# jkflying/opencalibration

Measured on AMD Instinct MI355X. Metric: images/sec end-to-end (extract+match+relax) on synthetic aerial grid; LM iters/sec, higher is better.
Workload: dtype f32 (extract) + fp4 0/1 bits, f32 accumulate, exact (match) + f64 (RANSAC, relax)

## Files before the change

### include/ochip.h

```cpp
#ifndef OCHIP_H
#define OCHIP_H

#include <stddef.h>
#include <stdint.h>

#ifdef __cplusplus
extern "C"
{
#endif

#define OCHIP_OK 0
#define OCHIP_EINVAL (-1)
#define OCHIP_ENOMEM (-2)
#define OCHIP_EHIP (-3)
#define OCHIP_ENODEV (-4)
#define OCHIP_ESTATE (-5)

#define OCHIP_DESC_WORDS64 8
#define OCHIP_DESC_BITS 486
#define OCHIP_NO_SECOND 0xFFFFu

    typedef struct ochip_ctx ochip_ctx;

    typedef struct ochip_pair
// ... 53 lines not shown
    {
        uint8_t *records;
        float *response;
        uint32_t *slot;
        uint32_t *num_sparse;
        uint8_t *conflict;
        uint32_t *subset;
        uint32_t *num_subset;
        uint8_t *subset_conflict;
        double subset_spacing;
    } ochip_feature_lists;
    int ochip_akaze_features(ochip_ctx *ctx, const uint8_t *images_bgr, uint32_t n_images, int width, int height, uint32_t max_kp,
                             double nms_radius, uint32_t *counts, const ochip_feature_lists *lists, int *work_wh);
    int ochip_akaze_features_dev(ochip_ctx *ctx, const uint8_t *images_bgr_dev, uint32_t n_images, int width, int height,
                                 uint32_t max_kp, double nms_radius, uint32_t *counts, const ochip_feature_lists *lists, int *work_wh);
    int ochip_feature_lists_from_keypoints(ochip_ctx *ctx, const float *kp6, const uint64_t *desc, const uint32_t *counts, uint32_t n_images,
                            uint32_t max_kp, int work_w, int work_h, double scale, double nms_radius,
                            const ochip_feature_lists *out);

    int ochip_synth_views_alloc(ochip_ctx *ctx, uint32_t n_images, int width, int height, uint8_t **images_dev);
    void ochip_synth_views_free(ochip_ctx *ctx, uint8_t *images_dev);
    int ochip_synth_views_read(ochip_ctx *ctx, const uint8_t *images_dev, uint32_t index, int width, int height,
                               uint8_t *host_out);
    int ochip_synth_render_views(ochip_ctx *ctx, uint8_t *images_dev, uint32_t first_image, uint32_t n_images, int width,
                                 int height, const double *cams, const double *model3, const double *plane2,
                                 const double *lattice3, uint32_t seed);

    int ochip_upload_keypoints(ochip_ctx *ctx, uint32_t image_id, const double *xy, uint32_t n, const double *model8);

    int ochip_upload_batch(ochip_ctx *ctx, uint32_t n_images, const uint32_t *counts, const uint64_t *desc_all,
// ... 352 lines not shown
```

### opencalibration_amd/capi.py

```python
import ctypes as C
import os

import numpy as np

_HERE = os.path.dirname(os.path.abspath(__file__))
LIB_PATH = os.path.join(_HERE, "libochip.so")

K_MATCH, K_RANSAC, K_RELAX_EVAL, K_RELAX_SOLVE, K_AKAZE = 0, 1, 2, 3, 4
NO_SECOND = 0xFFFF

PAIR_DTYPE = np.dtype([("image_1", np.uint32), ("image_2", np.uint32)])
MATCH_DTYPE = np.dtype([("best_k", np.uint32), ("best_count", np.uint16), ("second_count", np.uint16)])
RANSAC_JOB_DTYPE = np.dtype([("image_1", np.uint32), ("image_2", np.uint32), ("n", np.uint32), ("rng_state", np.uint32),
                             ("match_offset", np.uint64), ("eval_offset", np.uint64)])
RANSAC_MATCH_DTYPE = np.dtype([("k1", np.uint32), ("k2", np.uint32), ("count", np.uint16), ("reserved", np.uint16)])
RANSAC_RESULT_DTYPE = np.dtype([("H", np.float64, (9,)), ("score", np.float64), ("iterations", np.uint32), ("n_inliers", np.uint32),
                                ("improvements", np.uint32), ("reserved", np.uint32)])

EXPORTS = [
    "ochip_ctx_create", "ochip_ctx_destroy", "ochip_ctx_sibling", "ochip_ctx_attachment", "ochip_akaze_progress", "ochip_ctx_set_priority", "ochip_last_error", "ochip_device_info", "ochip_synchronize",
    "ochip_descriptors_reserve", "ochip_upload_descriptors", "ochip_descriptor_count",
    "ochip_match_batch", "ochip_match_launch", "ochip_match_fetch",
    "ochip_upload_keypoints", "ochip_ransac_homography_batch", "ochip_refit_homography_batch", "ochip_ransac_epipolar_batch",
    "ochip_upload_batch", "ochip_host_alloc", "ochip_host_free", "ochip_akaze_batch", "ochip_akaze_batch_dev", "ochip_akaze_features", "ochip_akaze_features_dev", "ochip_feature_lists_from_keypoints",
    "ochip_synth_views_alloc", "ochip_synth_views_free", "ochip_synth_render_views", "ochip_synth_views_read",
    "ochip_relax_problem_create", "ochip_relax_problem_destroy", "ochip_relax_set_cameras_constant",
    "ochip_relax_solve", "ochip_relax_get_state", "ochip_relax_set_shard", "ochip_relax_evaluate",
    "ochip_plane_setup_create", "ochip_plane_setup_override", "ochip_plane_setup_blocks", "ochip_plane_setup_destroy",
    "ochip_plane_chain_create", "ochip_plane_chain_run", "ochip_plane_chain_destroy",
    "ochip_relaxg_problem_create", "ochip_relaxg_problem_destroy", "ochip_relaxg_set_structure_only", "ochip_relaxg_solve",
    "ochip_relaxg_get_state", "ochip_relaxg_evaluate", "ochip_relaxg_set_exchange",
    "ochip_relaxp_problem_create", "ochip_relaxp_problem_destroy", "ochip_relaxp_set_structure_only", "ochip_relaxp_solve",
    "ochip_relaxp_get_state",
    "ochip_profile_reset", "ochip_profile_get", "ochip_match_work", "ochip_relax_work", "ochip_relax_memory", "ochip_work_counters",
    "ochip_debug_fp64", "ochip_debug_std_sort", "ochip_debug_lm_step", "ochip_debug_homography_fit4", "ochip_match_sort", "ochip_ransac_homography_batch_sorted", "ochip_edge_lists",
    "ochip_dense_index_create", "ochip_dense_index_destroy", "ochip_dense_match", "ochip_dense_link", "ochip_dense_triangulate",
    "ochip_rccl_unique_id", "ochip_rccl_comm_create", "ochip_rccl_comm_destroy", "ochip_rccl_comm_stats",
    "ochip_rccl_relax_exchange",
    "ochip_ortho_mesh_create", "ochip_ortho_mesh_destroy", "ochip_ortho_dsm", "ochip_ortho_thumbnail", "ochip_ortho_layers",
# ... 517 lines not shown
```

### opencalibration_amd/csrc/akaze.hip

```cpp
#include "ctx.hpp"

#include <algorithm>
#include <cmath>
#include <limits>
#include <cstring>
#include <type_traits>
#include <vector>

namespace
{

struct level_info
{
    int octave, w, h, sigma_size;
    float esigma;
    size_t off;
    int tile_off, tiles_x;
    int mask_off;
    int sup_off, sup_tx;
};

__device__ __forceinline__ int clampi(int v, int lo, int hi)
{
    return v < lo ? lo : (v > hi ? hi : v);
// ... 2621 lines not shown
            const float bx = x0 + ((float)(ci + di) + 0.5f + 0.6f * (hashf(id) - 0.5f)) * spacing;
            const float by = y0 + ((float)(cj + dj) + 0.5f + 0.6f * (hashf(id + 1) - 0.5f)) * spacing;
            const float amp = (0.25f + 0.5f * hashf(id + 2)) * ((hash32(id + 3) & 1) ? 1.0f : -1.0f);
            const float sg = spacing * (0.10f + 0.14f * hashf(id + 4));
            const float r2 = (gx - bx) * (gx - bx) + (gy - by) * (gy - by);
            v += amp * __expf(-r2 / (2.0f * sg * sg));
        }
    const float o = fminf(255.0f, fmaxf(0.0f, v * 255.0f));
    const uint8_t g = (uint8_t)o;
    uint8_t *p = out + ((size_t)blockIdx.z * w * h + (size_t)y * w + x) * 3;
    p[0] = g;
    p[1] = g;
    p[2] = g;
}

int akaze_run(ochip_ctx *ctx, const uint8_t *images_bgr, bool on_device, uint32_t n_images, int width, int height,
              uint32_t max_kp, float *kp6, uint64_t *desc, uint32_t *counts, int *work_wh,
              const ochip_feature_lists *lists = nullptr, double nms_radius = 8.0);

}

extern "C"
{

int ochip_akaze_batch(ochip_ctx *ctx, const uint8_t *images_bgr, uint32_t n_images, int width, int height,
                      uint32_t max_kp, float *kp6, uint64_t *desc, uint32_t *counts, int *work_wh)
{
    return akaze_run(ctx, images_bgr, false, n_images, width, height, max_kp, kp6, desc, counts, work_wh);
}

int ochip_akaze_batch_dev(ochip_ctx *ctx, const uint8_t *images_bgr_dev, uint32_t n_images, int width, int height,
                          uint32_t max_kp, float *kp6, uint64_t *desc, uint32_t *counts, int *work_wh)
{
    return akaze_run(ctx, images_bgr_dev, true, n_images, width, height, max_kp, kp6, desc, counts, work_wh);
}

int ochip_akaze_features(ochip_ctx *ctx, const uint8_t *images_bgr, uint32_t n_images, int width, int height, uint32_t max_kp,
                         double nms_radius, uint32_t *counts, const ochip_feature_lists *lists, int *work_wh)
// ... 173 lines not shown
        for (int k = 0; k < 16; k += 4)
            chains.push_back({2, 13 + k, -10 + (k / 4) * 5, -10, 0});
        for (size_t cidx = 0; cidx < chains.size(); cidx++)
            for (int ch = 0; ch < 3; ch++)
            {
                const ch_t &cc = chains[cidx];
                const unsigned int p0 = (unsigned int)((cc.i + 10) * 21 + (cc.j + 10));
                T.chain[3 * cidx + ch] = p0 | ((unsigned int)ch << 9) | ((unsigned int)cc.cls << 11) |
                                         ((unsigned int)cc.first_cell << 13) | ((unsigned int)cc.follows << 18);
            }
        return T;
    }();
    return G;
}

int akaze_run(ochip_ctx *ctx, const uint8_t *images_bgr, bool on_device, uint32_t n_images, int width, int height,
              uint32_t max_kp, float *kp6, uint64_t *desc, uint32_t *counts, int *work_wh, const ochip_feature_lists *lists,
              double nms_radius)
{
    if (!ctx || !counts || (n_images && (!images_bgr || (!lists && (!kp6 || !desc)))))
        return OCHIP_EINVAL;
    if (width <= 0 || height <= 0)
        return ochip_fail(ctx, OCHIP_EINVAL, "bad image size %d x %d", width, height);
    OCHIP_HIP(ctx, hipSetDevice(ctx->device));
    hipStream_t st = ctx->stream;
    const double scale = std::min(1.f, float(1600) / (float)std::max(width, height));
    const int W = (int)std::lrint(width * scale), H = (int)std::lrint(height * scale);
    if (work_wh)
    {
        work_wh[0] = W;
        work_wh[1] = H;
    }
    for (uint32_t i = 0; i < n_images; i++)
        counts[i] = 0;
    if (n_images == 0)
        return OCHIP_OK;
// ... 67 lines not shown
    unsigned char *d_dead = nullptr, *d_valid = nullptr;
    unsigned long long *d_desc = nullptr, *d_descc = nullptr;
    float *d_kpc = nullptr;
    unsigned int *d_counts = nullptr, *d_tile_counts = nullptr, *d_tile_base = nullptr, *d_tile_seq = nullptr;
    unsigned long long *d_mask = nullptr, *d_vmask = nullptr, *d_kmask = nullptr, *d_pmask = nullptr, *d_rmask = nullptr;
    unsigned int *d_found = nullptr;
    unsigned int *d_level_first = nullptr;
    unsigned int *d_turns = nullptr, *d_waiting = nullptr;
    unsigned int *d_wbase = nullptr, *d_live = nullptr, *d_nlive = nullptr;
    gather_tab *d_gtab = nullptr;
    const size_t src_px = (size_t)width * height;
    auto tiles = [&](int w, int h) { return dim3(8 * ((((w + BT_X - 1) / BT_X) * ((h + BT_Y - 1) / BT_Y) + 7) / 8), 1, B); };
    auto det_tiles = [&](int w, int h) { return dim3(8 * ((((w + BT_X - 1) / BT_X) * ((h + DT_Y - 1) / DT_Y) + 7) / 8), 1, B); };
    const dim3 tiles0 = tiles(W, H);
    const int n_tiles0 = ((W + BT_X - 1) / BT_X) * ((H + BT_Y - 1) / BT_Y);
    if (on_device)
        d_bgr = const_cast<uint8_t *>(images_bgr);
    else
        AK(up(ctx, allocs, &d_bgr, images_bgr, (size_t)B * src_px * 3));
    AK(up<uint8_t>(ctx, allocs, &d_gray, nullptr, (size_t)B * src_px + 4));
    AK(up<float>(ctx, allocs, &d_img, nullptr, (size_t)B * plane0));
    AK(up<float>(ctx, allocs, &d_flow, nullptr, (size_t)B * plane0));
    AK(up<float>(ctx, allocs, &d_ping, nullptr, (size_t)B * plane0));
    AK(up<unsigned int>(ctx, allocs, &d_pmax, nullptr, (size_t)B * n_tiles0));
    AK(up<float>(ctx, allocs, &d_Lt, nullptr, (size_t)B * img_stride));
    AK(up<float2>(ctx, allocs, &d_Lxy, nullptr, (size_t)B * img_stride));
    AK(up<float2>(ctx, allocs, &d_Fit, nullptr, (size_t)B * img_stride));
    AK(up<float>(ctx, allocs, &d_Rmax, nullptr, (size_t)B * img_stride));
    AK(up<float>(ctx, allocs, &d_kc, nullptr, B));
    AK(up<unsigned int>(ctx, allocs, &d_hmax, nullptr, B));
    AK(up<unsigned int>(ctx, allocs, &d_hist, nullptr, (size_t)B * 301));
    AK(up<unsigned int>(ctx, allocs, &d_ncand, nullptr, B));
    AK(up<cand_t>(ctx, allocs, &d_cands, nullptr, (size_t)B * max_cands));
    AK(up<unsigned char>(ctx, allocs, &d_dead, nullptr, (size_t)B * max_cands));
// ... 5 lines not shown
    AK(up<unsigned int>(ctx, allocs, &d_counts, nullptr, B));
    AK(up<unsigned int>(ctx, allocs, &d_tile_counts, nullptr, (size_t)B * n_tiles));
    AK(up<unsigned int>(ctx, allocs, &d_tile_base, nullptr, (size_t)B * n_tiles));
    AK(up<unsigned long long>(ctx, allocs, &d_mask, nullptr, (size_t)B * mask_stride));
    AK(up<unsigned long long>(ctx, allocs, &d_vmask, nullptr, (size_t)B * mask_stride));
    AK(up<unsigned long long>(ctx, allocs, &d_kmask, nullptr, (size_t)B * sup_stride));
    AK(up<unsigned long long>(ctx, allocs, &d_pmask, nullptr, (size_t)B * sup_stride));
    AK(up<unsigned long long>(ctx, allocs, &d_rmask, nullptr, (size_t)B * sup_stride));
    AK(up<unsigned int>(ctx, allocs, &d_turns, nullptr, (size_t)B * 2 * max_cands));
    AK(up<unsigned int>(ctx, allocs, &d_waiting, nullptr, (size_t)B * LV.n));
    AK(up<unsigned int>(ctx, allocs, &d_level_first, nullptr, (size_t)B * (LV.n + 1)));
    AK(up<unsigned int>(ctx, allocs, &d_found, nullptr, (size_t)B * max_cands));
    AK(up<unsigned int>(ctx, allocs, &d_wbase, nullptr, (size_t)B * mask_stride));
    AK(up<unsigned int>(ctx, allocs, &d_live, nullptr, (size_t)B * max_cands));
    AK(up<unsigned int>(ctx, allocs, &d_nlive, nullptr, B));
    {
        std::vector<std::pair<uint64_t, unsigned int>> keyed;
        keyed.reserve(n_tiles);
        auto spread = [](uint32_t v) {
            uint64_t x = v;
            x = (x | (x << 16)) & 0x0000FFFF0000FFFFull;
            x = (x | (x << 8)) & 0x00FF00FF00FF00FFull;
            x = (x | (x << 4)) & 0x0F0F0F0F0F0F0F0Full;
            x = (x | (x << 2)) & 0x3333333333333333ull;
            x = (x | (x << 1)) & 0x5555555555555555ull;
            return x;
        };
        for (int i = 0; i < LV.n; i++)
        {
            const level_info &l = LV.l[i];
            const int ty_n = (l.h + DT_Y - 1) / DT_Y;
            for (int ty = 0; ty < ty_n; ty++)
                for (int tx = 0; tx < l.tiles_x; tx++)
                    keyed.emplace_back(((uint64_t)i << 48) | spread((uint32_t)tx) | (spread((uint32_t)ty) << 1),
                                       (unsigned int)(l.tile_off + ty * l.tiles_x + tx));
        }
        std::sort(keyed.begin(), keyed.end());
        std::vector<unsigned int> seq(keyed.size());
        for (size_t i = 0; i < keyed.size(); i++)
            seq[i] = keyed[i].second;
        AK(up(ctx, allocs, &d_tile_seq, seq.data(), seq.size()));
    }
    {
        AK(up(ctx, allocs, &d_gtab, &host_gather_tab(), 1));
    }
    if (rc != OCHIP_OK)
    {
        cleanup();
        return rc;
    }
    auto grid2 = [&](int w, int h) { return dim3((w + 255) / 256, h, B); };
    auto taps_of = [](const std::vector<float> &k) {
        taps_t t{};
        t.n = (int)k.size();
        for (int i = 0; i < t.n && i < MAX_TAPS; i++)
            t.k[i] = k[i];
        return t;
    };
    const taps_t g1 = taps_of(gaussian_taps(1.0f)), g0 = taps_of(gaussian_taps(soffset));
    if (g1.n != 5 || g0.n != 9)
    {
        cleanup();
        return ochip_fail(ctx, OCHIP_EINVAL, "akaze: unexpected Gaussian kernel sizes %d / %d", g1.n, g0.n);
    }
    hipEvent_t e0, e1;
    ochip_prof_begin(ctx, OCHIP_K_AKAZE, &e0, &e1);

    const size_t n_px = (size_t)B * src_px;
    const bool resized = !(W == width && H == height);
    area_tab tx, ty;
    bool staged = false;
    if (resized)
    {
        tx = area_table(width, W, 1.0 / scale);
        ty = area_table(height, H, 1.0 / scale);
        staged = width % 4 == 0;
        for (int x0 = 0; x0 < W && staged; x0 += 256)
        {
            const int x1 = std::min(x0 + 256, W);
            const int c0 = tx.si[tx.off[x0]] & ~3, c1 = tx.si[tx.off[x1] - 1];
            staged = c1 - c0 + 1 <= RS_PITCH - 3;
            for (int x = x0; x < x1 && staged; x++)
                staged = tx.off[x + 1] - tx.off[x] <= RESIZE_MAX_TAPS;
        }
        for (int y0 = 0; y0 < H && staged; y0 += RESIZE_ROWS)
        {
            const int y1 = std::min(y0 + RESIZE_ROWS, H);
            staged = ty.si[ty.off[y1] - 1] - ty.si[ty.off[y0]] + 1 <= RS_ROWS;
        }
    }
    const bool fused_grey = staged && ((uintptr_t)d_bgr & 3) == 0;
    if (!fused_grey)
    {
        if (((uintptr_t)d_bgr & 3) == 0)
            hipLaunchKernelGGL(gray4_kernel, dim3((unsigned)(((n_px + 3) / 4 + 255) / 256)), dim3(256), 0, st,
                               (const uint32_t *)d_bgr, (uint32_t *)d_gray, n_px / 4);
        if (((uintptr_t)d_bgr & 3) != 0 || (n_px & 3))
        {
            const size_t first = ((uintptr_t)d_bgr & 3) ? 0 : (n_px & ~(size_t)3);
            hipLaunchKernelGGL(gray_kernel, dim3((unsigned)((n_px - first + 255) / 256)), dim3(256), 0, st, d_bgr + 3 * first,
                               d_gray + first, n_px - first);
        }
    }
    if (W == width && H == height)
        hipLaunchKernelGGL(to_float_kernel, dim3((unsigned)((B * plane0 + 255) / 256)), dim3(256), 0, st, d_gray, d_img,
                           B * plane0);
    else
    {
        int *xo, *xs, *yo, *ys;
        float *xa, *ya;
        AK(up(ctx, allocs, &xo, tx.off.data(), tx.off.size()));
        AK(up(ctx, allocs, &xs, tx.si.data(), tx.si.size()));
        AK(up(ctx, allocs, &xa, tx.alpha.data(), tx.alpha.size()));
        AK(up(ctx, allocs, &yo, ty.off.data(), ty.off.size()));
        AK(up(ctx, allocs, &ys, ty.si.data(), ty.si.size()));
        AK(up(ctx, allocs, &ya, ty.alpha.data(), ty.alpha.size()));
        if (rc != OCHIP_OK)
        {
            cleanup();
            return rc;
        }
        const dim3 rgrid((W + 255) / 256, (H + RESIZE_ROWS - 1) / RESIZE_ROWS, B);
        int most_taps = 0;
        for (int x = 0; x < W; x++)
            most_taps = std::max(most_taps, tx.off[x + 1] - tx.off[x]);
        const int half_up_cols = scale == 0.5 ? W - W % 16 : 0;
        if (fused_grey && most_taps <= 4)
            hipLaunchKernelGGL((resize_area_lds_kernel<true, 4>), rgrid, dim3(256), 0, st, (const uint8_t *)d_bgr, width, height, d_img,
                               W, H, xo, xs, xa, yo, ys, ya, half_up_cols);
        else if (fused_grey)
            hipLaunchKernelGGL((resize_area_lds_kernel<true, RESIZE_MAX_TAPS>), rgrid, dim3(256), 0, st, (const uint8_t *)d_bgr, width, height, d_img,
                               W, H, xo, xs, xa, yo, ys, ya, half_up_cols);
        else if (staged)
            hipLaunchKernelGGL((resize_area_lds_kernel<false, RESIZE_MAX_TAPS>), rgrid, dim3(256), 0, st, d_gray, width, height, d_img, W, H, xo, xs,
                               xa, yo, ys, ya, half_up_cols);
        else
            hipLaunchKernelGGL(resize_area_kernel, rgrid, dim3(256), 0, st, d_gray, width, height, d_img, W, H, xo, xs, xa, yo, ys,
                               ya, half_up_cols);
    }

// ... 302 lines not shown
            {
                std::fwrite(which ? hx.data() : hl.data(), 4, which ? hx.size() : hl.size(), f);
                std::fclose(f);
            }
    }
    hipLaunchKernelGGL(scan_tiles_kernel, dim3(B), dim3(256), 0, st, (const unsigned int *)d_tile_counts,
                       (const unsigned int *)d_tile_seq, n_tiles, d_tile_base, d_ncand);
    hipLaunchKernelGGL(collect_tiles_kernel, dim3((n_tiles + 4 * COLLECT_TPW - 1) / (4 * COLLECT_TPW), 1, B), dim3(256), 0, st, (const float *)d_Rmax,
                       (const float2 *)d_Fit, img_stride,
                       (const unsigned long long *)d_mask, mask_stride, LV, (const unsigned int *)d_tile_base, n_tiles, d_cands,
                       max_cands, (const unsigned int *)d_tile_counts);
    std::vector<unsigned int> ncand(B);
    OCHIP_HIP(ctx, hipMemcpyAsync(ncand.data(), d_ncand, B * 4, hipMemcpyDeviceToHost, st));
    OCHIP_HIP(ctx, ochip_stream_wait(ctx, st));
    ctx->akaze_readbacks.fetch_add(1, std::memory_order_release);
    unsigned int max_n = 0;
    for (uint32_t b = 0; b < B; b++)
    {
        if (ncand[b] > max_cands)
        {
            cleanup();
            return ochip_fail(ctx, OCHIP_ENOMEM, "image %u has %u extrema candidates; raise max_kp (candidate capacity %u)", b,
                              ncand[b], max_cands);
        }
        max_n = std::max(max_n, ncand[b]);
    }
    const int xcd_remap = 2;
    if (max_n > 0)
    {
        OCHIP_HIP(ctx, hipMemsetAsync(d_vmask, 0, (size_t)B * mask_stride * 8, st));
// ... 95 lines not shown
        if (counts[b] > max_kp)
        {
            rc = ochip_fail(ctx, OCHIP_ENOMEM, "image %u has %u keypoints, more than max_kp = %u", b, counts[b], max_kp);
            break;
        }
        most = std::max(most, counts[b]);
    }
    if (rc == OCHIP_OK && lists)
        rc = ochip::feature_lists_enqueue(ctx, &allocs, B, max_kp, d_kpc, d_descc, d_counts, most, W, H, scale, nms_radius, lists);
    else if (rc == OCHIP_OK && most > 0)
    {
        OCHIP_HIP(ctx, hipMemcpy2DAsync(kp6, (size_t)max_kp * 24, d_kpc, (size_t)max_kp * 24, (size_t)most * 24, B, hipMemcpyDeviceToHost, st));
        OCHIP_HIP(ctx, hipMemcpy2DAsync(desc, (size_t)max_kp * 64, d_descc, (size_t)max_kp * 64, (size_t)most * 64, B, hipMemcpyDeviceToHost, st));
    }
    if (rc != OCHIP_OK)
        for (uint32_t b = 0; b < B; b++)
            counts[b] = 0;
    cleanup();
    return rc;
#undef AK
}

}
```

### opencalibration_amd/csrc/ctx.hip

```cpp
#include "ctx.hpp"

#include <cstring>

static std::string g_create_error;

int ochip_fail(ochip_ctx *ctx, int code, const char *fmt, ...)
{
    char buf[512];
    va_list ap;
    va_start(ap, fmt);
    vsnprintf(buf, sizeof buf, fmt, ap);
    va_end(ap);
    if (ctx)
        ctx->error = buf;
    else
        g_create_error = buf;
    return code;
}

int ochip_ensure(ochip_ctx *ctx, void **ptr, size_t *cap, size_t bytes)
{
    if (bytes <= *cap)
        return OCHIP_OK;
    if (*ptr)
// ... 183 lines not shown
    for (void *b : bufs)
        if (b)
            (void)hipFree(b);
    for (void *b : ctx->scratch_dev)
        if (b)
            (void)hipFree(b);
    if (ctx->sym_jobs_dev)
        (void)hipFree(ctx->sym_jobs_dev);
    if (ctx->sym_part_dev)
        (void)hipFree(ctx->sym_part_dev);
    for (void *b : {ctx->desc_fp4_dev, ctx->desc_negpop_dev, ctx->desc_pop_dev})
        if (b)
            (void)hipFree(b);
    for (auto &b : ctx->dev_pool)
        (void)hipFree(b.first);
    for (auto &b : ctx->pinned_pool)
        (void)hipHostFree(b.first);
    for (auto &b : ctx->pinned_live)
        (void)hipHostFree(b.first);
    if (ctx->sync_event)
        (void)hipEventDestroy(ctx->sync_event);
    for (hipStream_t r : ctx->retired_streams)
        (void)hipStreamDestroy(r);
    if (ctx->stream)
        (void)hipStreamDestroy(ctx->stream);
    if (ctx->copy_stream)
        (void)hipStreamDestroy(ctx->copy_stream);
    delete ctx;
}

int ochip_ctx_set_priority(ochip_ctx *ctx, int high)
{
    if (!ctx)
        return OCHIP_EINVAL;
    if (ctx->stream_priority == (high ? 1 : 0))
        return OCHIP_OK;
    OCHIP_HIP(ctx, hipSetDevice(ctx->device));
    int least = 0, greatest = 0;
    OCHIP_HIP(ctx, hipDeviceGetStreamPriorityRange(&least, &greatest));
    OCHIP_HIP(ctx, hipStreamSynchronize(ctx->stream));
    hipStream_t s = nullptr;
    OCHIP_HIP(ctx, hipStreamCreateWithPriority(&s, hipStreamNonBlocking, high ? greatest : least));
    ctx->retired_streams.push_back(ctx->stream);
    ctx->stream = s;
    ctx->stream_priority = high ? 1 : 0;
    return OCHIP_OK;
}

int ochip_ctx_sibling(ochip_ctx *ctx, uint32_t index, ochip_ctx **out)
{
    if (!ctx || !out)
// ... 329 lines not shown
```

### opencalibration_amd/csrc/ctx.hpp

```cpp
#pragma once

#include <hip/hip_runtime.h>

#include <atomic>
#include <cstdarg>
#include <cstdio>
#include <mutex>
#include <string>
#include <vector>

#include "../../include/ochip.h"
#include "env.hpp"

struct ochip_profile_slot
{
    std::vector<std::pair<hipEvent_t, hipEvent_t>> pending;
    std::vector<std::pair<hipEvent_t, hipEvent_t>> free_list;
    uint64_t launches = 0;
    double total_ms = 0;
};

struct ochip_ctx
{
    int device = 0;
// ... 34 lines not shown
    uint64_t match_out_total = 0;
    void *ms_recs_dev = nullptr, *ms_seg_dev = nullptr, *ms_flag_dev = nullptr;
    size_t ms_recs_cap = 0, ms_seg_cap = 0, ms_flag_cap = 0;
    uint32_t ms_pairs = 0;
    void *sym_jobs_dev = nullptr, *sym_part_dev = nullptr;
    size_t sym_jobs_cap = 0, sym_part_cap = 0;
    void *desc_fp4_dev = nullptr, *desc_negpop_dev = nullptr, *desc_pop_dev = nullptr;
    size_t desc_fp4_cap = 0, desc_negpop_cap = 0, desc_pop_cap = 0;
    uint64_t fp4_valid = 0;

    void *scratch_dev[8] = {nullptr};
    size_t scratch_cap[8] = {0};

    std::vector<std::pair<void *, size_t>> pinned_live, pinned_pool;
    std::vector<std::pair<void *, size_t>> dev_pool;

    ochip_profile_slot prof[OCHIP_K_COUNT];
    uint64_t match_computed = 0, match_delivered = 0;
    double relax_mfma_flops = 0;
    uint64_t ransac_hyp_corr = 0, relax_blocks_jac = 0, relax_blocks_cost = 0;
    uint64_t relax_system_bytes = 0, relax_system_dense_bytes = 0, relax_system_unknowns = 0;

    std::vector<ochip_ctx *> siblings;
    std::mutex siblings_mutex;

    std::atomic<uint64_t> akaze_readbacks{0};

    void *attachment = nullptr;
    void (*attachment_destroy)(void *) = nullptr;
};


inline hipError_t ochip_stream_wait(ochip_ctx *ctx, hipStream_t st)
{
    if (!ctx->blocking_wait)
        return hipStreamSynchronize(st);
    if (!ctx->sync_event)
    {
        const hipError_t e = hipEventCreateWithFlags(&ctx->sync_event, hipEventBlockingSync | hipEventDisableTiming);
        if (e != hipSuccess)
            return e;
// ... 45 lines not shown
```

### opencalibration_amd/csrc/env.hpp

```cpp
#pragma once

#include <cstdlib>
#include <cstring>

inline bool ochip_env_list_has(const char *var, const char *name, bool one_means_all)
{
    const char *e = std::getenv(var);
    if (!e || !*e)
        return false;
    if (one_means_all && (std::strcmp(e, "1") == 0 || std::strcmp(e, "all") == 0))
        return true;
    const size_t len = std::strlen(name);
    for (const char *p = e; *p;)
    {
        const char *q = std::strchr(p, ',');
        const size_t n = q ? (size_t)(q - p) : std::strlen(p);
        if (n == len && std::strncmp(p, name, len) == 0)
            return true;
        p += n + (q ? 1 : 0);
    }
    return false;
}
inline bool ochip_verbose(const char *what)
{
    return ochip_env_list_has("OCHIP_VERBOSE", what, true);
}
inline bool ochip_test_hook(const char *name)
{
    return ochip_env_list_has("OCHIP_TEST_HOOKS", name, false);
}
```

### opencalibration_amd/csrc/host/extract_features.cpp

```cpp
#include "../env.hpp"
#include "extract_features.hpp"
#include "extract_slots.hpp"
#include "sort_like_std.hpp"

#include <algorithm>
#include <chrono>
#include <cmath>
#include <condition_variable>
#include <cstdio>
#include <cstdlib>
#include <cstring>
#include <deque>
#include <limits>
#include <mutex>
#include <thread>

#include <emmintrin.h>
#include <omp.h>

namespace opencalibration_amd
{

namespace
{
// ... 447 lines not shown
            double &out, t0;
            ~at_exit() { out = thread_cpu_now() - t0; }
        } record{driver_cpu[d], cpu0};
        {
            slot_hold hold(slots, ticket.id(), d, handover);
            if (trace)
                fprintf(stderr, "[extract] survey %llu driver %u: slot acquired\n", (unsigned long long)ticket.id(), d);
            {
                std::lock_guard<std::mutex> lk(mu);
                if (!started)
                {
                    started = true;
                    t_first_slot = std::chrono::steady_clock::now();
                }
            }
            for (;;)
            {
                uint32_t c = 0;
                bool go = false;
                {
                    std::unique_lock<std::mutex> lk(mu);
                    if (stagger)
                        while (fail.empty() && next_chunk < n_chunks)
                        {
                            bool other = false;
                            for (uint32_t o = 0; o < n_drivers; o++)
                                if (o != d && in_first_phase[o])
                                {
                                    if (ochip_akaze_progress(ctxs[o]) != progress_at_start[o])
                                        in_first_phase[o] = 0;
// ... 9 lines not shown
                        c = next_chunk++;
                        go = true;
                        if (stagger)
                        {
                            progress_at_start[d] = ochip_akaze_progress(dctx);
                            in_first_phase[d] = 1;
                        }
                    }
                }
                if (!go)
                    break;
                if (c + 1 == n_chunks && handover == extract_slots::order::slot)
                    ticket.retire();
                if (trace)
                    fprintf(stderr, "[extract] survey %llu driver %u: chunk %u of %u\n", (unsigned long long)ticket.id(), d, c, n_chunks);
                const int sb = slots.take_buffer(d);
                const int which = BPS * (int)d + sb;
                chunk_buffers &b = bufs[which];
                int rc = OCHIP_OK;
                if (!shape_buffer(dctx, slots.at(d, sb), b))
                    rc = OCHIP_ENOMEM;
                b.first = c * chunk;
                b.n = std::min(chunk, n_images - b.first);
                int wh[2];
                const uint8_t *src = images_bgr + (size_t)b.first * image_bytes;
                if (rc != OCHIP_OK)
                    ;
                else if (device_tail)
                    rc = images_on_device ? ochip_akaze_features_dev(dctx, src, b.n, width, height, max_keypoints, nms_pixel_radius,
                                                                     b.counts.data(), &b.lists, wh)
                                          : ochip_akaze_features(dctx, src, b.n, width, height, max_keypoints, nms_pixel_radius,
                                                                 b.counts.data(), &b.lists, wh);
                else
                    rc = images_on_device ? ochip_akaze_batch_dev(dctx, src, b.n, width, height, max_keypoints, b.kp, b.desc,
                                                                  b.counts.data(), wh)
                                          : ochip_akaze_batch(dctx, src, b.n, width, height, max_keypoints, b.kp, b.desc,
                                                              b.counts.data(), wh);
                std::unique_lock<std::mutex> lk(mu);
                in_first_phase[d] = 0;
                if (rc != OCHIP_OK)
                {
                    if (fail.empty())
                        fail = std::string("ochip_akaze_batch: ") + ochip_last_error(dctx);
                    if (trace)
                        fprintf(stderr, "[extract] survey %llu driver %u: chunk %u failed (%s)\n", (unsigned long long)ticket.id(), d, c,
                                ochip_last_error(dctx));
                    lk.unlock();
                    cv.notify_all();
                    slots.return_buffer(d, sb);
                    ticket.retire();
                    break;
                }
                ready.push_back(which);
                cv.notify_all();
            }
        }
        if (trace)
            fprintf(stderr, "[extract] survey %llu driver %u: slot released\n", (unsigned long long)ticket.id(), d);
        std::unique_lock<std::mutex> lk(mu);
        drivers_done++;
        cv.notify_all();
    };
    std::vector<std::thread> drivers;
    for (uint32_t d = 0; d < n_drivers; d++)
        drivers.emplace_back(driver, d);
    std::chrono::steady_clock::time_point t_last_final = t_enter;

    for (;;)
    {
        int which;
// ... 123 lines not shown
```

### opencalibration_amd/csrc/host/extract_slots.hpp

```cpp
#pragma once

#include <condition_variable>
#include <cstddef>
#include <cstdint>
#include <mutex>
#include <set>

namespace opencalibration_amd
{

class extract_slots
{
  public:
    static constexpr uint32_t MAX_SLOTS = 8;
    static constexpr int BUFFERS_PER_SLOT = 3;
    enum class order
    {
        slot,
        survey,
        none
    };
    struct buffer
    {
        void *block[2] = {nullptr, nullptr};
// ... 49 lines not shown
    {
        std::unique_lock<std::mutex> lk(mu_);
        int b = -1;
        cv_.wait(lk, [&] {
            for (int i = 0; i < BUFFERS_PER_SLOT; i++)
                if (!slot_[d].buf[i].busy)
                {
                    b = i;
                    return true;
                }
            return false;
        });
        slot_[d].buf[b].busy = true;
        return b;
    }
    void return_buffer(uint32_t d, int b)
    {
        {
            std::lock_guard<std::mutex> lk(mu_);
            slot_[d].buf[b].busy = false;
        }
        cv_.notify_all();
    }
    buffer &at(uint32_t d, int b) { return slot_[d].buf[b]; }

  private:
    struct slot
    {
        bool held = false;
        uint64_t holder = 0;
// ... 44 lines not shown
```

Measured before the change: 3896.

## Split AKAZE extraction into begin/finish to overlap chunks and cache lookup tables

Extraction now runs in two steps. A begin call enqueues a chunk and records an event, and a finish call waits on that event later. This lets the host driver start the next chunk while the previous chunk's result copies are still draining. The tile-order sequence, gather table and resize tables are now cached on the context instead of being rebuilt and uploaded every batch, which removes per-chunk host sorting and small uploads. The cost is extra state: a pending-chunk limit, event recycling, and callback-driven collection, all of which raise the risk of ordering or buffer-lifetime bugs.

```diff
diff --git a/include/ochip.h b/include/ochip.h
--- a/include/ochip.h
+++ b/include/ochip.h
@@ -91,6 +91,12 @@
                              double nms_radius, uint32_t *counts, const ochip_feature_lists *lists, int *work_wh);
     int ochip_akaze_features_dev(ochip_ctx *ctx, const uint8_t *images_bgr_dev, uint32_t n_images, int width, int height,
                                  uint32_t max_kp, double nms_radius, uint32_t *counts, const ochip_feature_lists *lists, int *work_wh);
+    typedef struct ochip_akaze_job ochip_akaze_job;
+    int ochip_akaze_begin(ochip_ctx *ctx, const uint8_t *images_bgr, int images_on_device, uint32_t n_images, int width, int height,
+                          uint32_t max_kp, double nms_radius, float *kp6, uint64_t *desc, uint32_t *counts,
+                          const ochip_feature_lists *lists, int *work_wh, void (*stream_drained)(void *), void *arg,
+                          ochip_akaze_job **job);
+    int ochip_akaze_finish(ochip_ctx *ctx, ochip_akaze_job *job);
     int ochip_feature_lists_from_keypoints(ochip_ctx *ctx, const float *kp6, const uint64_t *desc, const uint32_t *counts, uint32_t n_images,
                             uint32_t max_kp, int work_w, int work_h, double scale, double nms_radius,
                             const ochip_feature_lists *out);
diff --git a/opencalibration_amd/capi.py b/opencalibration_amd/capi.py
--- a/opencalibration_amd/capi.py
+++ b/opencalibration_amd/capi.py
@@ -22,7 +22,7 @@
     "ochip_descriptors_reserve", "ochip_upload_descriptors", "ochip_descriptor_count",
     "ochip_match_batch", "ochip_match_launch", "ochip_match_fetch",
     "ochip_upload_keypoints", "ochip_ransac_homography_batch", "ochip_refit_homography_batch", "ochip_ransac_epipolar_batch",
-    "ochip_upload_batch", "ochip_host_alloc", "ochip_host_free", "ochip_akaze_batch", "ochip_akaze_batch_dev", "ochip_akaze_features", "ochip_akaze_features_dev", "ochip_feature_lists_from_keypoints",
+    "ochip_upload_batch", "ochip_host_alloc", "ochip_host_free", "ochip_akaze_batch", "ochip_akaze_batch_dev", "ochip_akaze_features", "ochip_akaze_features_dev", "ochip_akaze_begin", "ochip_akaze_finish", "ochip_feature_lists_from_keypoints",
     "ochip_synth_views_alloc", "ochip_synth_views_free", "ochip_synth_render_views", "ochip_synth_views_read",
     "ochip_relax_problem_create", "ochip_relax_problem_destroy", "ochip_relax_set_cameras_constant",
     "ochip_relax_solve", "ochip_relax_get_state", "ochip_relax_set_shard", "ochip_relax_evaluate",
diff --git a/opencalibration_amd/csrc/akaze.hip b/opencalibration_amd/csrc/akaze.hip
--- a/opencalibration_amd/csrc/akaze.hip
+++ b/opencalibration_amd/csrc/akaze.hip
@@ -2659,14 +2659,65 @@
     p[2] = g;
 }
 
+int akaze_begin(ochip_ctx *ctx, const uint8_t *images_bgr, bool on_device, uint32_t n_images, int width, int height,
+                uint32_t max_kp, float *kp6, uint64_t *desc, uint32_t *counts, int *work_wh, const ochip_feature_lists *lists,
+                double nms_radius, void (*stream_drained)(void *), void *arg, ochip_akaze_job **job);
+
 int akaze_run(ochip_ctx *ctx, const uint8_t *images_bgr, bool on_device, uint32_t n_images, int width, int height,
               uint32_t max_kp, float *kp6, uint64_t *desc, uint32_t *counts, int *work_wh,
-              const ochip_feature_lists *lists = nullptr, double nms_radius = 8.0);
-
-}
+              const ochip_feature_lists *lists = nullptr, double nms_radius = 8.0)
+{
+    ochip_akaze_job *job = nullptr;
+    const int rc = akaze_begin(ctx, images_bgr, on_device, n_images, width, height, max_kp, kp6, desc, counts, work_wh, lists,
+                               nms_radius, nullptr, nullptr, &job);
+    return rc != OCHIP_OK ? rc : ochip_akaze_finish(ctx, job);
+}
+
+}
+
+struct ochip_akaze_job
+{
+    hipEvent_t done = nullptr;
+    uint32_t *counts = nullptr;
+    uint32_t n_images = 0;
+};
 
 extern "C"
 {
+
+int ochip_akaze_begin(ochip_ctx *ctx, const uint8_t *images_bgr, int images_on_device, uint32_t n_images, int width, int height,
+                      uint32_t max_kp, double nms_radius, float *kp6, uint64_t *desc, uint32_t *counts,
+                      const ochip_feature_lists *lists, int *work_wh, void (*stream_drained)(void *), void *arg,
+                      ochip_akaze_job **job)
+{
+    if (!job)
+        return OCHIP_EINVAL;
+    *job = nullptr;
+    if (lists && (!lists->records || !lists->response || !lists->slot || !lists->num_sparse || !lists->conflict))
+        return OCHIP_EINVAL;
+    return akaze_begin(ctx, images_bgr, images_on_device != 0, n_images, width, height, max_kp, kp6, desc, counts, work_wh, lists,
+                       nms_radius, stream_drained, arg, job);
+}
+
+int ochip_akaze_finish(ochip_ctx *ctx, ochip_akaze_job *job)
+{
+    if (!ctx)
+        return OCHIP_EINVAL;
+    if (!job)
+        return OCHIP_OK;
+    const hipError_t e = hipEventSynchronize(job->done);
+    ctx->akaze_events.push_back(job->done);
+    ctx->akaze_pending--;
+    int rc = OCHIP_OK;
+    if (e != hipSuccess)
+    {
+        for (uint32_t b = 0; b < job->n_images; b++)
+            job->counts[b] = 0;
+        rc = ochip_fail(ctx, OCHIP_EHIP, "akaze: the chunk's result copies failed: %s", hipGetErrorString(e));
+    }
+    delete job;
+    return rc;
+}
 
 int ochip_akaze_batch(ochip_ctx *ctx, const uint8_t *images_bgr, uint32_t n_images, int width, int height,
                       uint32_t max_kp, float *kp6, uint64_t *desc, uint32_t *counts, int *work_wh)
@@ -2870,12 +2921,126 @@
     return G;
 }
 
-int akaze_run(ochip_ctx *ctx, const uint8_t *images_bgr, bool on_device, uint32_t n_images, int width, int height,
-              uint32_t max_kp, float *kp6, uint64_t *desc, uint32_t *counts, int *work_wh, const ochip_feature_lists *lists,
-              double nms_radius)
-{
+int akaze_tables_ensure(ochip_ctx *ctx, int width, int height, int W, int H, double scale, const levels_dev &LV, int n_tiles)
+{
+    auto &T = ctx->akaze_tab;
+    hipStream_t st = ctx->stream;
+    if (!T.gather)
+    {
+        void *g = nullptr;
+        if (hipMalloc(&g, sizeof(gather_tab)) != hipSuccess)
+            return ochip_fail(ctx, OCHIP_ENOMEM, "device allocation of %zu bytes failed in akaze", sizeof(gather_tab));
+        if (hipMemcpyAsync(g, &host_gather_tab(), sizeof(gather_tab), hipMemcpyHostToDevice, st) != hipSuccess ||
+            ochip_stream_wait(ctx, st) != hipSuccess)
+        {
+            (void)hipFree(g);
+            return ochip_fail(ctx, OCHIP_EHIP, "hipMemcpy failed in akaze");
+        }
+        T.gather = g;
+    }
+    if (T.block && T.width == width && T.height == height && T.W == W && T.H == H && T.n_tiles == n_tiles)
+        return OCHIP_OK;
+    OCHIP_HIP(ctx, ochip_stream_wait(ctx, st));
+    if (T.block)
+        OCHIP_HIP(ctx, hipFree(T.block));
+    T.block = nullptr;
+    T.width = T.height = T.W = T.H = 0;
+    std::vector<unsigned int> seq;
+    {
+        std::vector<std::pair<uint64_t, unsigned int>> keyed;
+        keyed.reserve(n_tiles);
+        auto spread = [](uint32_t v) {
+            uint64_t x = v;
+            x = (x | (x << 16)) & 0x0000FFFF0000FFFFull;
+            x = (x | (x << 8)) & 0x00FF00FF00FF00FFull;
+            x = (x | (x << 4)) & 0x0F0F0F0F0F0F0F0Full;
+            x = (x | (x << 2)) & 0x3333333333333333ull;
+            x = (x | (x << 1)) & 0x5555555555555555ull;
+            return x;
+        };
+        for (int i = 0; i < LV.n; i++)
+        {
+            const level_info &l = LV.l[i];
+            const int ty_n = (l.h + DT_Y - 1) / DT_Y;
+            for (int ty = 0; ty < ty_n; ty++)
+                for (int tx = 0; tx < l.tiles_x; tx++)
+                    keyed.emplace_back(((uint64_t)i << 48) | spread((uint32_t)tx) | (spread((uint32_t)ty) << 1),
+                                       (unsigned int)(l.tile_off + ty * l.tiles_x + tx));
+        }
+        std::sort(keyed.begin(), keyed.end());
+        seq.resize(keyed.size());
+        for (size_t i = 0; i < keyed.size(); i++)
+            seq[i] = keyed[i].second;
+    }
+    const bool resized = !(W == width && H == height);
+    area_tab tx, ty;
+    bool staged = false;
+    int most_taps = 0;
+    if (resized)
+    {
+        tx = area_table(width, W, 1.0 / scale);
+        ty = area_table(height, H, 1.0 / scale);
+        staged = width % 4 == 0;
+        for (int x0 = 0; x0 < W && staged; x0 += 256)
+        {
+            const int x1 = std::min(x0 + 256, W);
+            const int c0 = tx.si[tx.off[x0]] & ~3, c1 = tx.si[tx.off[x1] - 1];
+            staged = c1 - c0 + 1 <= RS_PITCH - 3;
+            for (int x = x0; x < x1 && staged; x++)
+                staged = tx.off[x + 1] - tx.off[x] <= RESIZE_MAX_TAPS;
+        }
+        for (int y0 = 0; y0 < H && staged; y0 += RESIZE_ROWS)
+        {
+            const int y1 = std::min(y0 + RESIZE_ROWS, H);
+            staged = ty.si[ty.off[y1] - 1] - ty.si[ty.off[y0]] + 1 <= RS_ROWS;
+        }
+        for (int x = 0; x < W; x++)
+            most_taps = std::max(most_taps, tx.off[x + 1] - tx.off[x]);
+    }
+    const void *part[7] = {seq.data(), tx.off.data(), tx.si.data(), tx.alpha.data(), ty.off.data(), ty.si.data(), ty.alpha.data()};
+    const size_t len[7] = {seq.size(), tx.off.size(), tx.si.size(), tx.alpha.size(), ty.off.size(), ty.si.size(), ty.alpha.size()};
+    size_t bytes = 0;
+    for (int k = 0; k < 7; k++)
+    {
+        T.off[k] = bytes;
+        bytes += (std::max<size_t>(len[k], 1) * 4 + 255) / 256 * 256;
+    }
+    std::vector<unsigned char> host(bytes, 0);
+    for (int k = 0; k < 7; k++)
+        if (len[k])
+            std::memcpy(host.data() + T.off[k], part[k], len[k] * 4);
+    void *d = nullptr;
+    if (hipMalloc(&d, bytes) != hipSuccess)
+        return ochip_fail(ctx, OCHIP_ENOMEM, "device allocation of %zu bytes failed in akaze", bytes);
+    if (hipMemcpyAsync(d, host.data(), bytes, hipMemcpyHostToDevice, st) != hipSuccess || ochip_stream_wait(ctx, st) != hipSuccess)
+    {
+        (void)hipFree(d);
+        return ochip_fail(ctx, OCHIP_EHIP, "hipMemcpy failed in akaze");
+    }
+    T.block = d;
+    T.bytes = bytes;
+    T.width = width;
+    T.height = height;
+    T.W = W;
+    T.H = H;
+    T.n_tiles = n_tiles;
+    T.most_taps = most_taps;
+    T.resized = resized;
+    T.staged = staged;
+    return OCHIP_OK;
+}
+
+int akaze_begin(ochip_ctx *ctx, const uint8_t *images_bgr, bool on_device, uint32_t n_images, int width, int height,
+                uint32_t max_kp, float *kp6, uint64_t *desc, uint32_t *counts, int *work_wh, const ochip_feature_lists *lists,
+                double nms_radius, void (*stream_drained)(void *), void *arg, ochip_akaze_job **job)
+{
+    *job = nullptr;
     if (!ctx || !counts || (n_images && (!images_bgr || (!lists && (!kp6 || !desc)))))
         return OCHIP_EINVAL;
+    if (ctx->akaze_pending && ctx->pool_stream != ctx->stream)
+        return ochip_fail(ctx, OCHIP_ESTATE, "akaze: the context's stream was replaced while a chunk is pending");
+    if (ctx->akaze_pending >= 2)
+        return ochip_fail(ctx, OCHIP_ESTATE, "akaze: %u chunks pending on the context; finish one first", ctx->akaze_pending);
     if (width <= 0 || height <= 0)
         return ochip_fail(ctx, OCHIP_EINVAL, "bad image size %d x %d", width, height);
     OCHIP_HIP(ctx, hipSetDevice(ctx->device));
@@ -2973,10 +3138,20 @@
     auto det_tiles = [&](int w, int h) { return dim3(8 * ((((w + BT_X - 1) / BT_X) * ((h + DT_Y - 1) / DT_Y) + 7) / 8), 1, B); };
     const dim3 tiles0 = tiles(W, H);
     const int n_tiles0 = ((W + BT_X - 1) / BT_X) * ((H + BT_Y - 1) / BT_Y);
+    bool drained_told = false;
+    auto drained = [&]() {
+        if (stream_drained && !drained_told)
+            stream_drained(arg);
+        drained_told = true;
+    };
     if (on_device)
         d_bgr = const_cast<uint8_t *>(images_bgr);
     else
+    {
         AK(up(ctx, allocs, &d_bgr, images_bgr, (size_t)B * src_px * 3));
+        if (rc == OCHIP_OK)
+            drained();
+    }
     AK(up<uint8_t>(ctx, allocs, &d_gray, nullptr, (size_t)B * src_px + 4));
     AK(up<float>(ctx, allocs, &d_img, nullptr, (size_t)B * plane0));
     AK(up<float>(ctx, allocs, &d_flow, nullptr, (size_t)B * plane0));
@@ -3012,35 +3187,13 @@
     AK(up<unsigned int>(ctx, allocs, &d_wbase, nullptr, (size_t)B * mask_stride));
     AK(up<unsigned int>(ctx, allocs, &d_live, nullptr, (size_t)B * max_cands));
     AK(up<unsigned int>(ctx, allocs, &d_nlive, nullptr, B));
-    {
-        std::vector<std::pair<uint64_t, unsigned int>> keyed;
-        keyed.reserve(n_tiles);
-        auto spread = [](uint32_t v) {
-            uint64_t x = v;
-            x = (x | (x << 16)) & 0x0000FFFF0000FFFFull;
-            x = (x | (x << 8)) & 0x00FF00FF00FF00FFull;
-            x = (x | (x << 4)) & 0x0F0F0F0F0F0F0F0Full;
-            x = (x | (x << 2)) & 0x3333333333333333ull;
-            x = (x | (x << 1)) & 0x5555555555555555ull;
-            return x;
-        };
-        for (int i = 0; i < LV.n; i++)
-        {
-            const level_info &l = LV.l[i];
-            const int ty_n = (l.h + DT_Y - 1) / DT_Y;
-            for (int ty = 0; ty < ty_n; ty++)
-                for (int tx = 0; tx < l.tiles_x; tx++)
-                    keyed.emplace_back(((uint64_t)i << 48) | spread((uint32_t)tx) | (spread((uint32_t)ty) << 1),
-                                       (unsigned int)(l.tile_off + ty * l.tiles_x + tx));
-        }
-        std::sort(keyed.begin(), keyed.end());
-        std::vector<unsigned int> seq(keyed.size());
-        for (size_t i = 0; i < keyed.size(); i++)
-            seq[i] = keyed[i].second;
-        AK(up(ctx, allocs, &d_tile_seq, seq.data(), seq.size()));
-    }
-    {
-        AK(up(ctx, allocs, &d_gtab, &host_gather_tab(), 1));
+    AK(akaze_tables_ensure(ctx, width, height, W, H, scale, LV, n_tiles));
+    const auto &tab = ctx->akaze_tab;
+    auto tab_part = [&](int k) { return (void *)((unsigned char *)tab.block + tab.off[k]); };
+    if (rc == OCHIP_OK)
+    {
+        d_tile_seq = (unsigned int *)tab_part(0);
+        d_gtab = (gather_tab *)tab.gather;
     }
     if (rc != OCHIP_OK)
     {
@@ -3065,28 +3218,7 @@
     ochip_prof_begin(ctx, OCHIP_K_AKAZE, &e0, &e1);
 
     const size_t n_px = (size_t)B * src_px;
-    const bool resized = !(W == width && H == height);
-    area_tab tx, ty;
-    bool staged = false;
-    if (resized)
-    {
-        tx = area_table(width, W, 1.0 / scale);
-        ty = area_table(height, H, 1.0 / scale);
-        staged = width % 4 == 0;
-        for (int x0 = 0; x0 < W && staged; x0 += 256)
-        {
-            const int x1 = std::min(x0 + 256, W);
-            const int c0 = tx.si[tx.off[x0]] & ~3, c1 = tx.si[tx.off[x1] - 1];
-            staged = c1 - c0 + 1 <= RS_PITCH - 3;
-            for (int x = x0; x < x1 && staged; x++)
-                staged = tx.off[x + 1] - tx.off[x] <= RESIZE_MAX_TAPS;
-        }
-        for (int y0 = 0; y0 < H && staged; y0 += RESIZE_ROWS)
-        {
-            const int y1 = std::min(y0 + RESIZE_ROWS, H);
-            staged = ty.si[ty.off[y1] - 1] - ty.si[ty.off[y0]] + 1 <= RS_ROWS;
-        }
-    }
+    const bool staged = tab.staged;
     const bool fused_grey = staged && ((uintptr_t)d_bgr & 3) == 0;
     if (!fused_grey)
     {
@@ -3105,23 +3237,11 @@
                            B * plane0);
     else
     {
-        int *xo, *xs, *yo, *ys;
-        float *xa, *ya;
-        AK(up(ctx, allocs, &xo, tx.off.data(), tx.off.size()));
-        AK(up(ctx, allocs, &xs, tx.si.data(), tx.si.size()));
-        AK(up(ctx, allocs, &xa, tx.alpha.data(), tx.alpha.size()));
-        AK(up(ctx, allocs, &yo, ty.off.data(), ty.off.size()));
-        AK(up(ctx, allocs, &ys, ty.si.data(), ty.si.size()));
-        AK(up(ctx, allocs, &ya, ty.alpha.data(), ty.alpha.size()));
-        if (rc != OCHIP_OK)
-        {
-            cleanup();
-            return rc;
-        }
+        const int *xo = (const int *)tab_part(1), *xs = (const int *)tab_part(2), *yo = (const int *)tab_part(4),
+                  *ys = (const int *)tab_part(5);
+        const float *xa = (const float *)tab_part(3), *ya = (const float *)tab_part(6);
         const dim3 rgrid((W + 255) / 256, (H + RESIZE_ROWS - 1) / RESIZE_ROWS, B);
-        int most_taps = 0;
-        for (int x = 0; x < W; x++)
-            most_taps = std::max(most_taps, tx.off[x + 1] - tx.off[x]);
+        const int most_taps = tab.most_taps;
         const int half_up_cols = scale == 0.5 ? W - W % 16 : 0;
         if (fused_grey && most_taps <= 4)
             hipLaunchKernelGGL((resize_area_lds_kernel<true, 4>), rgrid, dim3(256), 0, st, (const uint8_t *)d_bgr, width, height, d_img,
@@ -3454,6 +3574,7 @@
     OCHIP_HIP(ctx, hipMemcpyAsync(ncand.data(), d_ncand, B * 4, hipMemcpyDeviceToHost, st));
     OCHIP_HIP(ctx, ochip_stream_wait(ctx, st));
     ctx->akaze_readbacks.fetch_add(1, std::memory_order_release);
+    drained();
     unsigned int max_n = 0;
     for (uint32_t b = 0; b < B; b++)
     {
@@ -3579,10 +3700,39 @@
         OCHIP_HIP(ctx, hipMemcpy2DAsync(desc, (size_t)max_kp * 64, d_descc, (size_t)max_kp * 64, (size_t)most * 64, B, hipMemcpyDeviceToHost, st));
     }
     if (rc != OCHIP_OK)
+    {
         for (uint32_t b = 0; b < B; b++)
             counts[b] = 0;
-    cleanup();
-    return rc;
+        cleanup();
+        return rc;
+    }
+    hipEvent_t done = nullptr;
+    if (!ctx->akaze_events.empty())
+    {
+        done = ctx->akaze_events.back();
+        ctx->akaze_events.pop_back();
+    }
+    else if (hipEventCreateWithFlags(&done, (ctx->blocking_wait ? hipEventBlockingSync : 0) | hipEventDisableTiming) != hipSuccess)
+        done = nullptr;
+    if (!done || hipEventRecord(done, st) != hipSuccess || st != ctx->stream)
+    {
+        if (done)
+            ctx->akaze_events.push_back(done);
+        for (uint32_t b = 0; b < B; b++)
+            counts[b] = 0;
+        cleanup();
+        return ochip_fail(ctx, OCHIP_EHIP, "akaze: no event behind the chunk's result copies");
+    }
+    for (auto &a : allocs)
+        ochip_pool_put(ctx, a.first, a.second);
+    ctx->pool_stream = st;
+    ctx->akaze_pending++;
+    ochip_akaze_job *j = new ochip_akaze_job();
+    j->done = done;
+    j->counts = counts;
+    j->n_images = B;
+    *job = j;
+    return OCHIP_OK;
 #undef AK
 }
 
diff --git a/opencalibration_amd/csrc/ctx.hip b/opencalibration_amd/csrc/ctx.hip
--- a/opencalibration_amd/csrc/ctx.hip
+++ b/opencalibration_amd/csrc/ctx.hip
@@ -221,6 +221,11 @@
             (void)hipFree(b);
     for (auto &b : ctx->dev_pool)
         (void)hipFree(b.first);
+    for (void *b : {ctx->akaze_tab.block, ctx->akaze_tab.gather})
+        if (b)
+            (void)hipFree(b);
+    for (hipEvent_t e : ctx->akaze_events)
+        (void)hipEventDestroy(e);
     for (auto &b : ctx->pinned_pool)
         (void)hipHostFree(b.first);
     for (auto &b : ctx->pinned_live)
@@ -242,6 +247,8 @@
         return OCHIP_EINVAL;
     if (ctx->stream_priority == (high ? 1 : 0))
         return OCHIP_OK;
+    if (ctx->akaze_pending)
+        return ochip_fail(ctx, OCHIP_ESTATE, "set_priority: %u extraction chunks are pending on the context", ctx->akaze_pending);
     OCHIP_HIP(ctx, hipSetDevice(ctx->device));
     int least = 0, greatest = 0;
     OCHIP_HIP(ctx, hipDeviceGetStreamPriorityRange(&least, &greatest));
diff --git a/opencalibration_amd/csrc/ctx.hpp b/opencalibration_amd/csrc/ctx.hpp
--- a/opencalibration_amd/csrc/ctx.hpp
+++ b/opencalibration_amd/csrc/ctx.hpp
@@ -72,6 +72,7 @@
 
     std::vector<std::pair<void *, size_t>> pinned_live, pinned_pool;
     std::vector<std::pair<void *, size_t>> dev_pool;
+    hipStream_t pool_stream = nullptr;
 
     ochip_profile_slot prof[OCHIP_K_COUNT];
     uint64_t match_computed = 0, match_delivered = 0;
@@ -83,6 +84,17 @@
     std::mutex siblings_mutex;
 
     std::atomic<uint64_t> akaze_readbacks{0};
+    uint32_t akaze_pending = 0;
+    std::vector<hipEvent_t> akaze_events;
+    struct akaze_tables
+    {
+        int width = 0, height = 0, W = 0, H = 0;
+        void *block = nullptr;
+        size_t bytes = 0, off[7] = {0, 0, 0, 0, 0, 0, 0};
+        int n_tiles = 0, most_taps = 0;
+        bool resized = false, staged = false;
+        void *gather = nullptr;
+    } akaze_tab;
 
     void *attachment = nullptr;
     void (*attachment_destroy)(void *) = nullptr;
diff --git a/opencalibration_amd/csrc/env.hpp b/opencalibration_amd/csrc/env.hpp
--- a/opencalibration_amd/csrc/env.hpp
+++ b/opencalibration_amd/csrc/env.hpp
@@ -29,3 +29,7 @@
 {
     return ochip_env_list_has("OCHIP_TEST_HOOKS", name, false);
 }
+inline bool ochip_extract_chunk_pending()
+{
+    return !ochip_test_hook("finish_before_begin");
+}
diff --git a/opencalibration_amd/csrc/host/extract_features.cpp b/opencalibration_amd/csrc/host/extract_features.cpp
--- a/opencalibration_amd/csrc/host/extract_features.cpp
+++ b/opencalibration_amd/csrc/host/extract_features.cpp
@@ -485,6 +485,36 @@
                     t_first_slot = std::chrono::steady_clock::now();
                 }
             }
+            struct pending_chunk
+            {
+                ochip_akaze_job *job = nullptr;
+                int sb = -1, which = -1;
+                uint32_t c = 0;
+            } pending;
+            auto collect = [&]() -> bool {
+                if (pending.which < 0)
+                    return true;
+                const int rc = ochip_akaze_finish(dctx, pending.job);
+                const int sb = pending.sb, which = pending.which;
+                pending = pending_chunk{};
+                std::unique_lock<std::mutex> lk(mu);
+                if (rc != OCHIP_OK)
+                {
+                    if (fail.empty())
+                        fail = std::string("ochip_akaze_batch: ") + ochip_last_error(dctx);
+                    lk.unlock();
+                    cv.notify_all();
+                    slots.return_buffer(d, sb);
+                    return false;
+                }
+                ready.push_back(which);
+                cv.notify_all();
+                return true;
+            };
+            bool collected_ok = true;
+            auto collect_from_begin = [&]() { collected_ok = collect() && collected_ok; };
+            using collect_fn = decltype(collect_from_begin);
+            const bool keep_pending = ochip_extract_chunk_pending();
             for (;;)
             {
                 uint32_t c = 0;
@@ -524,7 +554,12 @@
                     ticket.retire();
                 if (trace)
                     fprintf(stderr, "[extract] survey %llu driver %u: chunk %u of %u\n", (unsigned long long)ticket.id(), d, c, n_chunks);
-                const int sb = slots.take_buffer(d);
+                int sb = slots.try_take_buffer(d);
+                if (sb < 0)
+                {
+                    collected_ok = collect() && collected_ok;
+                    sb = slots.take_buffer(d);
+                }
                 const int which = BPS * (int)d + sb;
                 chunk_buffers &b = bufs[which];
                 int rc = OCHIP_OK;
@@ -534,18 +569,22 @@
                 b.n = std::min(chunk, n_images - b.first);
                 int wh[2];
                 const uint8_t *src = images_bgr + (size_t)b.first * image_bytes;
-                if (rc != OCHIP_OK)
-                    ;
-                else if (device_tail)
-                    rc = images_on_device ? ochip_akaze_features_dev(dctx, src, b.n, width, height, max_keypoints, nms_pixel_radius,
-                                                                     b.counts.data(), &b.lists, wh)
-                                          : ochip_akaze_features(dctx, src, b.n, width, height, max_keypoints, nms_pixel_radius,
-                                                                 b.counts.data(), &b.lists, wh);
-                else
-                    rc = images_on_device ? ochip_akaze_batch_dev(dctx, src, b.n, width, height, max_keypoints, b.kp, b.desc,
-                                                                  b.counts.data(), wh)
-                                          : ochip_akaze_batch(dctx, src, b.n, width, height, max_keypoints, b.kp, b.desc,
-                                                              b.counts.data(), wh);
+                ochip_akaze_job *job = nullptr;
+                if (rc == OCHIP_OK)
+                    rc = ochip_akaze_begin(dctx, src, images_on_device ? 1 : 0, b.n, width, height, max_keypoints, nms_pixel_radius,
+                                           device_tail ? nullptr : b.kp, device_tail ? nullptr : b.desc, b.counts.data(),
+                                           device_tail ? &b.lists : nullptr, wh,
+                                           [](void *f) { (*static_cast<collect_fn *>(f))(); }, &collect_from_begin, &job);
+                collected_ok = collect() && collected_ok;
+                if (rc == OCHIP_OK)
+                {
+                    pending.job = job;
+                    pending.sb = sb;
+                    pending.which = which;
+                    pending.c = c;
+                    if (!keep_pending)
+                        collected_ok = collect() && collected_ok;
+                }
                 std::unique_lock<std::mutex> lk(mu);
                 in_first_phase[d] = 0;
                 if (rc != OCHIP_OK)
@@ -561,9 +600,15 @@
                     ticket.retire();
                     break;
                 }
-                ready.push_back(which);
-                cv.notify_all();
+                if (!collected_ok)
+                {
+                    lk.unlock();
+                    ticket.retire();
+                    break;
+                }
             }
+            if (!collect())
+                ticket.retire();
         }
         if (trace)
             fprintf(stderr, "[extract] survey %llu driver %u: slot released\n", (unsigned long long)ticket.id(), d);
diff --git a/opencalibration_amd/csrc/host/extract_slots.hpp b/opencalibration_amd/csrc/host/extract_slots.hpp
--- a/opencalibration_amd/csrc/host/extract_slots.hpp
+++ b/opencalibration_amd/csrc/host/extract_slots.hpp
@@ -87,6 +87,17 @@
         slot_[d].buf[b].busy = true;
         return b;
     }
+    int try_take_buffer(uint32_t d)
+    {
+        std::lock_guard<std::mutex> lk(mu_);
+        for (int i = 0; i < BUFFERS_PER_SLOT; i++)
+            if (!slot_[d].buf[i].busy)
+            {
+                slot_[d].buf[i].busy = true;
+                return i;
+            }
+        return -1;
+    }
     void return_buffer(uint32_t d, int b)
     {
         {
```

New measurement: 3871. About the same (-0.7%).
